# sisl/MADRL

Hardware: AMD Instinct MI355X
Metric: env-steps/sec at fixed batch (PursuitEvade 16x16, 8v30) (higher is better)
Workload: dtype u8/int32 grid state, f32 observations, f64 reward arithmetic; 1 GPU; PursuitEvade 16x16, 8 pursuers / 30 evaders, obs_range 7, rectangle_map, surround, n_catch 2, flatten, local reward, 65536 envs per GPU, horizon 500; envs_per_gpu=65536, envs_total=65536, parallelism=env-sharded x1, streams_per_gpu=2, rccl_ranks=1

## Files before the change

### madrl_amd/csrc/pursuit_wave.hpp

```cpp
#pragma once

#include <type_traits>

#include "common.hpp"

namespace madrl {
namespace pw {

#ifndef MADRL_PW_WAVES
#define MADRL_PW_WAVES 5
#endif
#define MADRL_PW_OCC __attribute__((amdgpu_waves_per_eu(S::OCC, S::OCC)))

constexpr uint32_t SENT = 0xFFFFFFFFu;
constexpr uint32_t CAUGHT = 0x10000u;

struct WaveDev {
    int32_t n_catch, surround, reward_global, sample_maps, n_maps, max_steps, auto_reset;
    int32_t fmap_stride;
    int32_t max_opponents;
    int32_t reverse;
    uint32_t k0, k1, gid_base;
    double catchr, term_pursuit, urgency, cw;
    int64_t n_envs;
    const uint32_t *fmaps;
    const float *vtab;
    const int32_t *pending;
    const uint32_t *cnt_tmpl;
    const uint32_t *slot_tab;
    const double *cw_env;
    const double *catchr_env;
    uint8_t *state;
    uint32_t *flags;
    uint32_t *zmask;
};

struct WaveIO {
    const uint8_t *mask;
    const int32_t *inj_pos;
    const int32_t *inj_map;
    const int32_t *actions;
    const int32_t *inj_eact;
    float *obs;
    float *rew;
    uint8_t *done;
    int32_t *removed;
    int32_t flex;
    int32_t control_evaders;
    const float *obs_prev;
};

__device__ __forceinline__ double sload_f64(const double *p, int64_t index) {
    return ((const __attribute__((address_space(4))) double *)(uint64_t)p)[index];
}

struct KArgs {
    WaveDev d;
    WaveIO io;
};
typedef const __attribute__((address_space(4))) KArgs *KArgsPtr;
__device__ __forceinline__ KArgsPtr cold_args() { return kernargs<KArgs>(); }
__device__ __forceinline__ int32_t pending_count(int64_t env, int k) {
    const int32_t *pend = cold_args()->d.pending;
    return ((const __attribute__((address_space(4))) int32_t *)(uint64_t)pend)[2 * env + k];
}

template <int XS_, int YS_, int P_, int E_, int R_, int FLATTEN_>
struct Shape {
    static constexpr int XS = XS_, YS = YS_, P = P_, E = E_, A = P_ + E_, R = R_, FLATTEN = FLATTEN_;
    static constexpr int OFF = (R - 1) / 2;
    static constexpr int PAD = OFF > 1 ? OFF : 1;
    static constexpr int GW = YS + 2 * PAD;
    static constexpr int GH = XS + 2 * PAD;
    static constexpr int GSZ = (GH * GW + 3) / 4 * 4;
    static constexpr int D = FLATTEN ? 3 * R * R + 1 : 4 * R * R;
    static constexpr int DV = D / 4;
    static constexpr int NQ = P * DV;
    static constexpr int NS = (NQ + 63) / 64;
    static constexpr int MWORDS = 1;
    static constexpr int OCC = NS <= 5 ? MADRL_PW_WAVES : (MADRL_PW_WAVES < 4 ? MADRL_PW_WAVES : 4);
    static constexpr int X_FILL = 3 * GSZ;
    static constexpr int X_SKIP = 3 * GSZ + 1;
    static constexpr int X_ID = 3 * GSZ + 2;
    static constexpr int X_VTAB = (X_ID + P + 3) / 4 * 4;
    static constexpr int NVT = 72;
    static constexpr int X_NEED = X_VTAB + NVT;
    static constexpr int X_OBSV = X_NEED + (XS * YS + 3) / 4;
    static constexpr int LDS_DWORDS = X_OBSV + (P + 3) / 4 * 4;
    static constexpr int NGW = (E + 31) / 32 > 0 ? (E + 31) / 32 : 1;
    static constexpr int NTW = (A + 31) / 32;
    static constexpr int OFF_GONE = (16 + 2 * A + 3) / 4 * 4;
    static constexpr int OFF_TERM = OFF_GONE + 4 * NGW;
    static constexpr int REC_BYTES = (OFF_TERM + 4 * NTW + 15) / 16 * 16;
    static constexpr int REC_DW = REC_BYTES / 4;
    static_assert(REC_DW <= 64, "the whole record must fit one dword per lane");
    static_assert(A <= 64, "one wavefront per env: n_pursuers + n_evaders must fit 64 lanes");
    static_assert(R % 2 == 1, "odd obs_range only (even ranges run on the generic kernel)");
    static_assert(D % 4 == 0, "observation row must be a whole number of float4");
    static_assert(LDS_DWORDS * 4 <= 64 * 1024, "LDS budget");
    static_assert(NS <= 8, "stale-zero mask: one bit per slot in each byte of the lane's mask dword");
    static constexpr bool LIVE = false;
    static constexpr bool TO = false;
    static constexpr bool TABLED = false;
    static constexpr int X_TAB = 0;
};

template <int XS_, int YS_, int P_, int E_, int R_, int FLATTEN_>
struct LShape : Shape<XS_, YS_, P_, E_, R_, FLATTEN_> {
    static constexpr bool LIVE = true;
};
constexpr int NOT_HERE = 0xFF;

template <int XS_, int YS_, int P_, int E_, int R_, int FLATTEN_>
struct TShape : Shape<XS_, YS_, P_, E_, R_, FLATTEN_> {
    static constexpr bool TO = true;
};
template <int XS_, int YS_, int P_, int E_, int R_, int FLATTEN_>
struct TLShape : LShape<XS_, YS_, P_, E_, R_, FLATTEN_> {
    static constexpr bool TO = true;
};

__device__ __forceinline__ double pairwise8(const double *r) {
    return ((r[0] + r[1]) + (r[2] + r[3])) + ((r[4] + r[5]) + (r[6] + r[7]));
}

template <int P>
__device__ __forceinline__ double np_sum_regs(const double (&a)[P]) {
    if constexpr (P < 8) {
        double res = 0.0;
#pragma unroll
        for (int i = 0; i < P; ++i) res += a[i];
        return res;
    } else {
        double r[8];
#pragma unroll
        for (int i = 0; i < 8; ++i) r[i] = a[i];
        constexpr int LIM = P - (P % 8);
#pragma unroll
        for (int i = 8; i < LIM; i += 8) {
#pragma unroll
            for (int k = 0; k < 8; ++k) r[k] += a[i + k];
        }
        double res = pairwise8(r);
#pragma unroll
        for (int i = LIM; i < P; ++i) res += a[i];
        return res;
    }
}

template <int P>
__device__ __forceinline__ double np_sum_first(const double (&a)[P], int n) {
    double res = 0.0;
    if (n < 8) {
#pragma unroll
        for (int i = 0; i < (P < 8 ? P : 7); ++i)
            if (i < n) res += a[i];
        return res;
    }
    if constexpr (P >= 8) {
        double r[8];
#pragma unroll
        for (int i = 0; i < 8; ++i) r[i] = a[i];
        const int lim = n - (n % 8);
#pragma unroll
        for (int i = 8; i + 8 <= P; i += 8) {
            if (i < lim) {
#pragma unroll
                for (int k = 0; k < 8; ++k) r[k] += a[i + k];
            }
        }
        res = pairwise8(r);
#pragma unroll
        for (int i = 8; i < P; ++i)
            if (i >= lim && i < n) res += a[i];
    }
    return res;
}

typedef float v4f_t __attribute__((ext_vector_type(4)));
template <int I, int N, class F>
__device__ __forceinline__ void static_for(F &&f) {
    if constexpr (I < N) {
        f(std::integral_constant<int, I>{});
        static_for<I + 1, N>(f);
    }
}
template <int OFF>
__device__ __forceinline__ void store_slot_masked(const void *base, uint32_t voff, uint32_t v0, uint32_t v1, uint32_t v2, uint32_t v3,
                                                  v4f_t val, uint64_t m0, uint64_t m1, uint64_t m2, uint64_t m3, uint64_t m_nt) {
    uint64_t sv;
    asm volatile("s_mov_b64 %0, exec\n\t"
                 "s_mov_b64 exec, %1\n\tglobal_store_dword %6, %7, %12 offset:%13\n\t"
                 "s_mov_b64 exec, %2\n\tglobal_store_dword %6, %8, %12 offset:%13+4\n\t"
                 "s_mov_b64 exec, %3\n\tglobal_store_dword %6, %9, %12 offset:%13+8\n\t"
                 "s_mov_b64 exec, %4\n\tglobal_store_dword %6, %10, %12 offset:%13+12\n\t"
                 "s_mov_b64 exec, %5\n\tglobal_store_dwordx4 %6, %11, %12 offset:%13 nt\n\t"
                 "s_mov_b64 exec, %0\n\ts_nop 0"
                 : "=&s"(sv) : "s"(m0), "s"(m1), "s"(m2), "s"(m3), "s"(m_nt), "v"(voff), "v"(v0), "v"(v1), "v"(v2), "v"(v3), "v"(val),
                   "s"(base), "n"(OFF));
}
__device__ __forceinline__ uint32_t quad_or(uint32_t v) {
    v |= (uint32_t)__builtin_amdgcn_update_dpp(0, (int)v, 0xB1, 0xF, 0xF, true);
    v |= (uint32_t)__builtin_amdgcn_update_dpp(0, (int)v, 0x4E, 0xF, 0xF, true);
    return v;
}

__device__ __forceinline__ void prefetch3(uint32_t &r0, uint32_t &r1, uint32_t &r2, const void *b0, uint32_t o0, const void *b1, uint32_t o1,
                                          const void *b2, uint32_t o2) {
    asm volatile("s_nop 4\n\tglobal_load_dword %0, %3, %4\n\tglobal_load_dword %1, %5, %6\n\tglobal_load_dword %2, %7, %8"
                 : "=&v"(r0), "=&v"(r1), "=&v"(r2) : "v"(o0), "s"(b0), "v"(o1), "s"(b1), "v"(o2), "s"(b2));
}
template <int N>
__device__ __forceinline__ void prefetch_wait(uint32_t &r0, uint32_t &r1, uint32_t &r2) {
    static_assert(N >= 0 && N < 64, "vmcnt is a 6-bit field");
    asm volatile("s_waitcnt vmcnt(%3)" : "+v"(r0), "+v"(r1), "+v"(r2) : "n"(N) : "memory");
}

template <int LN>
__device__ __forceinline__ void put_lane(uint32_t &w, uint32_t v) {
    const uint32_t sv = (uint32_t)__builtin_amdgcn_readfirstlane((int)v);
    asm("v_writelane_b32 %0, %1, %2" : "+v"(w) : "s"(sv), "n"(LN));
}
template <int LN, int END>
__device__ __forceinline__ void put_zero_from(uint32_t &w) {
    if constexpr (LN < END) {
        put_lane<LN>(w, 0u);
        put_zero_from<LN + 1, END>(w);
    }
}

template <class S, int NT>
struct Fill {
    static constexpr int NEEDW = (S::XS * S::YS + 3) / 4;
    static constexpr int TABW = S::TABLED ? 2 * S::DV : 0;
    static constexpr int J_MAP = (S::GSZ + NT - 1) / NT;
    static constexpr int J_NEED = 2 * J_MAP;
    static constexpr int J_VT = J_NEED + (NEEDW + NT - 1) / NT;
    static constexpr int J_TAB = J_VT + (S::NVT + NT - 1) / NT;
    static constexpr int J_END = J_TAB + (TABW + NT - 1) / NT;
    static constexpr int first(int j) { return j < J_MAP ? 0 : j < J_NEED ? J_MAP : j < J_VT ? J_NEED : j < J_TAB ? J_VT : J_TAB; }
    static constexpr int words(int j) { return j < J_NEED ? S::GSZ : j < J_VT ? NEEDW : j < J_TAB ? S::NVT : TABW; }
};
template <class S, int NT, int J>
__device__ __forceinline__ uint32_t fill_load(uint32_t utid, const uint32_t *cnt, const uint32_t *map, const uint32_t *vtab, const uint32_t *tab) {
    using F = Fill<S, NT>;
    constexpr int t = J - F::first(J), n = F::words(J);
    const uint32_t k = utid + (uint32_t)(NT * t);
    const uint32_t kc = (NT * (t + 1) <= n) ? k : (k < (uint32_t)n ? k : (uint32_t)n - 1u);
    if constexpr (J < F::J_MAP) return cnt[kc];
    else if constexpr (J < F::J_NEED) return map[kc];
    else if constexpr (J < F::J_VT) return map[(uint32_t)S::GSZ + kc];
    else if constexpr (J < F::J_TAB) return vtab[kc];
    else return tab[kc];
}
template <class S, int NT, int J, bool FIRST>
__device__ __forceinline__ void fill_store(uint32_t *L, uint32_t utid, uint32_t v) {
    using F = Fill<S, NT>;
    constexpr int t = J - F::first(J), n = F::words(J);
    const uint32_t k = utid + (uint32_t)(NT * t);
    if ((NT * (t + 1) <= n) || k < (uint32_t)n) {
        if constexpr (J < F::J_MAP) {
            L[S::GSZ + k] = v;
            L[2 * S::GSZ + k] = v;
        } else if constexpr (J < F::J_NEED) L[k] = v;
        else if constexpr (J < F::J_VT) L[S::X_NEED + k] = v;
        else if constexpr (J < F::J_TAB) L[S::X_VTAB + k] = v;
        else L[S::X_TAB + k] = v;
    }
    if constexpr (FIRST && J == F::J_MAP) {
        if (utid == 0u) {
            L[S::X_FILL] = v;
            L[S::X_SKIP] = SENT;
        }
    }
}
template <int N>
__device__ __forceinline__ void staged_wait(uint32_t *a) {
    if constexpr (N >= 8) {
        asm volatile("" : "+v"(a[N - 1]), "+v"(a[N - 2]), "+v"(a[N - 3]), "+v"(a[N - 4]), "+v"(a[N - 5]), "+v"(a[N - 6]), "+v"(a[N - 7]), "+v"(a[N - 8]));
        staged_wait<N - 8>(a);
    } else if constexpr (N >= 4) {
        asm volatile("" : "+v"(a[N - 1]), "+v"(a[N - 2]), "+v"(a[N - 3]), "+v"(a[N - 4]));
        staged_wait<N - 4>(a);
    } else if constexpr (N >= 2) {
        asm volatile("" : "+v"(a[N - 1]), "+v"(a[N - 2]));
        staged_wait<N - 2>(a);
    } else if constexpr (N == 1) {
        asm volatile("" : "+v"(a[0]));
    }
}
template <class S, int NT, int J0, int J1, int CAP, bool FIRST>
__device__ __forceinline__ void fill_trips(uint32_t *L, uint32_t utid, const uint32_t *cnt, const uint32_t *map, const uint32_t *vtab, const uint32_t *tab) {
    if constexpr (J0 < J1) {
        constexpr int JB = J0 + CAP < J1 ? J0 + CAP : J1;
        uint32_t st[JB - J0];
        static_for<J0, JB>([&](auto jc) {
            if constexpr (decltype(jc)::value == JB - 1) __builtin_amdgcn_sched_barrier(0);
            st[decltype(jc)::value - J0] = fill_load<S, NT, decltype(jc)::value>(utid, cnt, map, vtab, tab);
        });
        staged_wait<JB - J0>(st);
        static_for<J0, JB>([&](auto jc) { fill_store<S, NT, decltype(jc)::value, FIRST>(L, utid, st[decltype(jc)::value - J0]); });
        fill_trips<S, NT, JB, J1, CAP, FIRST>(L, utid, cnt, map, vtab, tab);
    }
}
constexpr int FILL_FIRST = 56, FILL_BATCH = 16;

#ifndef MADRL_ABLATE
#define MADRL_ABLATE 0
#endif
#ifndef MADRL_PW_EXP
#define MADRL_PW_EXP 0
#endif

template <class S, int MODE, bool INJECT, bool CTRL = false>
__global__ __launch_bounds__(64) MADRL_PW_OCC void pursuit_wave_kernel(const WaveDev d, const WaveIO io) {
    static_assert(!CTRL || (S::E >= S::P && (MODE == 0 || INJECT)), "evader control: n_evaders >= n_pursuers, flexible instantiation");
    static_assert(!CTRL || !S::LIVE, "evader control has no per-env agent counts");
    static_assert(!S::TO || (MODE == 1 && INJECT && !CTRL), "the two-buffer step: the flexible step kernel only");
    constexpr int P = S::P, E = S::E, A = S::A, GW = S::GW, PAD = S::PAD, GSZ = S::GSZ, NS = S::NS;
    __shared__ __attribute__((aligned(16))) uint32_t L[S::LDS_DWORDS];
    const int lane = threadIdx.x;
    const uint32_t ulane = threadIdx.x;
    const bool is_p = lane < P;
    const int eslot = lane - P;

#if MADRL_PW_EXP & 4
    if (d.n_envs > 0) return;
#endif
    using F = Fill<S, 64>;
    const int n_envs = (int)d.n_envs, stride = (int)gridDim.x;
    if (n_envs <= 0) return;
    auto phys = [&](int e) -> int64_t { return (int64_t)(d.reverse ? n_envs - 1 - e : e); };
    const uint32_t *const vtab_u = reinterpret_cast<const uint32_t *>(d.vtab);
    constexpr int ROOM = FILL_FIRST - 6 * NS - 3;
    constexpr int JF = F::J_END < (ROOM > 4 ? ROOM : 4) ? F::J_END : (ROOM > 4 ? ROOM : 4);
    const uint32_t rec_off = (ulane < (uint32_t)S::REC_DW ? ulane : (uint32_t)S::REC_DW - 1u) * 4u;
    const uint32_t act_off = (ulane < (uint32_t)P ? ulane : (uint32_t)P - 1u) * 4u;
    uint32_t st[JF], sraw[6 * NS];
    static_for<0, JF>([&](auto jc) { st[decltype(jc)::value] = fill_load<S, 64, decltype(jc)::value>(ulane, d.cnt_tmpl, d.fmaps, vtab_u, nullptr); });
#pragma unroll
    for (int k = 0; k < 6 * NS; ++k) sraw[k] = d.slot_tab[64u * k + ulane];
    uint32_t cur_rec, cur_zm;
    int cur_act = 4;
    __builtin_amdgcn_sched_barrier(0);
    {
        const int64_t env0 = phys((int)blockIdx.x < n_envs ? (int)blockIdx.x : n_envs - 1);
        cur_rec = *reinterpret_cast<const uint32_t *>(d.state + env0 * (int64_t)S::REC_BYTES + rec_off);
        if constexpr (MODE == 1) cur_act = *reinterpret_cast<const int *>(reinterpret_cast<const char *>(io.actions + env0 * P) + act_off);
        cur_zm = d.zmask[env0 * 64 + ulane];
    }
    asm volatile("" : "+v"(cur_rec), "+v"(cur_act), "+v"(cur_zm));
    staged_wait<6 * NS>(sraw);
    staged_wait<JF>(st);
    static_for<0, JF>([&](auto jc) { fill_store<S, 64, decltype(jc)::value, true>(L, ulane, st[decltype(jc)::value]); });
    fill_trips<S, 64, JF, F::J_END, FILL_BATCH, true>(L, ulane, d.cnt_tmpl, d.fmaps, vtab_u, nullptr);
    if (lane < P) L[S::X_ID + lane] = __float_as_uint((float)((double)lane / (double)P));
    if (ulane >= (uint32_t)S::REC_DW) cur_rec = 0u;
    if (!is_p) cur_act = 4;
    int s_cst[NS][4];
    int s_rel3[NS];
    int s_src[NS];
#pragma unroll
    for (int s = 0; s < NS; ++s) {
#pragma unroll
        for (int k = 0; k < 4; ++k) s_cst[s][k] = (int)sraw[6 * s + k] * 4;
        s_rel3[s] = (int)sraw[6 * s + 4];
        s_src[s] = (int)sraw[6 * s + 5] * 4;
    }
    int cached_map = 0;
    int cached_np = P;
    const uint8_t *need_tab = reinterpret_cast<const uint8_t *>(&L[S::X_NEED]);
    uint32_t *const layer = &L[is_p ? GSZ : 2 * GSZ];
    const int rec_src0 = (lane >= 4 ? 2 * (lane - 4) : 0) * 4, rec_src1 = rec_src0 + 4;

    auto isP = [&]() { return fresh(lane) < P; };
    auto isE = [&]() { return (unsigned)(fresh(lane) - P) < (unsigned)E; };
    auto isAgent = [&]() { return fresh(lane) < A; };
    auto fetch_rec = [&](int64_t env) -> uint32_t {
        return (fresh(lane) < S::REC_DW) ? uniform_ptr(reinterpret_cast<const uint32_t *>(d.state + env * (int64_t)S::REC_BYTES))[ulane] : 0u;
    };
    auto fetch_act = [&](int64_t env) -> int {
        if constexpr (MODE == 1) return isP() ? uniform_ptr(io.actions + env * P)[ulane] : 4;
        else return 4;
    };
    auto fetch_zm = [&](int64_t env) -> uint32_t { return uniform_ptr(d.zmask + env * 64)[ulane]; };
    wave_sync();
#if MADRL_PW_EXP & 8
    if (d.n_envs > 0) { if (s_cst[0][0] + s_cst[NS - 1][3] + s_rel3[0] + s_src[NS - 1] + (int)cur_rec == 0x12345) io.rew[0] = 1.f; return; }
#endif

    constexpr bool PIPE = (MODE == 1) && !INJECT && !(MADRL_ABLATE & (1 | 8 | 16 | 64));
    constexpr int VM_PER_ENV = 5 * NS + 6;
    static_assert(!PIPE || VM_PER_ENV < 64, "vmcnt range");
    for (int e = blockIdx.x; e < n_envs; e += stride) {
        const int64_t env = phys(e);
        const bool has_next = e + stride < n_envs;
        const int64_t nenv = phys(has_next ? e + stride : e);
        uint32_t nxt_rec = 0, nxt_zm = 0xFFFFFFFFu;
        int nxt_act = 4;
        uint32_t pf_rec, pf_act, pf_zm;
        if constexpr (PIPE) {
            prefetch3(pf_rec, pf_act, pf_zm, d.state + nenv * (int64_t)S::REC_BYTES, rec_off, io.actions + nenv * P, act_off,
                      d.zmask + nenv * 64, ulane * 4u);
        } else {
#if MADRL_ABLATE & 64
            nxt_rec = cur_rec ^ (uint32_t)(fresh(lane) == 0);
            nxt_act = cur_act;
#else
            if (has_next) {
                nxt_rec = fetch_rec(nenv);
                nxt_act = fetch_act(nenv);
                nxt_zm = fetch_zm(nenv);
            }
#endif
        }
        bool skip = false;
        if constexpr (MODE == 0) skip = (io.mask != nullptr && io.mask[env] == 0);
        if (!skip) {
            uint32_t tick = __builtin_amdgcn_readlane(cur_rec, 0);
            int32_t tstep = (int32_t)__builtin_amdgcn_readlane(cur_rec, 1);
            int32_t map_id = (int32_t)__builtin_amdgcn_readlane(cur_rec, 2);
            const uint32_t xyw = (uint32_t)__shfl((int)cur_rec, 4 + (lane >> 1));
            const uint32_t xy = (lane & 1) ? (xyw >> 16) : (xyw & 0xFFFFu);
            int x = (int)(xy & 0xFF), y = (int)(xy >> 8);
            uint64_t gone = (uint32_t)__builtin_amdgcn_readlane(cur_rec, S::OFF_GONE / 4);
            if constexpr (S::NGW > 1) gone |= (uint64_t)(uint32_t)__builtin_amdgcn_readlane(cur_rec, S::OFF_GONE / 4 + 1) << 32;
            uint64_t term = (uint32_t)__builtin_amdgcn_readlane(cur_rec, S::OFF_TERM / 4);
            if constexpr (S::NTW > 1) term |= (uint64_t)(uint32_t)__builtin_amdgcn_readlane(cur_rec, S::OFF_TERM / 4 + 1) << 32;
            const uint32_t gid = d.gid_base + (uint32_t)env;
            const uint32_t k0 = fresh_s(d.k0), k1 = fresh_s(d.k1);
            int np = P, ne = E;
            if constexpr (S::LIVE) {
                const bool here = x != NOT_HERE;
                np = __popcll(__builtin_amdgcn_ballot_w64(isP() && here));
                ne = __popcll(__builtin_amdgcn_ballot_w64(isE() && here));
                if (!here) {
                    x = 0;
                    y = 0;
                }
            }
            auto isLP = [&]() {
                if constexpr (S::LIVE) return fresh(lane) < np;
                else return isP();
            };
            bool do_reset = (MODE == 0);
            uint32_t done_bits = 0;
            float rew_out = 0.0f;
            int n_removed = 0;
            bool alive = isLP() || (isE() && !((gone >> eslot) & 1ull));
            int cell = (x + PAD) * GW + y + PAD;

            auto load_map = [&](int mid) {
                if (cached_map == mid) return;
                const KArgsPtr ka = cold_args();
                fill_trips<S, 64, F::J_MAP, F::J_VT, FILL_BATCH, false>(L, ulane, nullptr, ka->d.fmaps + (int64_t)mid * ka->d.fmap_stride, nullptr, nullptr);
                cached_map = mid;
                wave_sync();
            };
            load_map(map_id);

            if constexpr (MODE == 1) {
                const bool e_alive = alive && !isP();
                if (e_alive) atomicAdd(&layer[cell], 1u);
                wave_sync();
                int kpre = 0;
                if (isP()) {
                    const int dxm = (x > 0) ? GW : 0, dxp = (x < S::XS - 1) ? GW : 0;
                    const int dym = (y > 0) ? 1 : 0, dyp = (y < S::YS - 1) ? 1 : 0;
                    const uint32_t *ec = &L[2 * GSZ];
                    kpre = (int)(ec[cell - dxm] + ec[cell + dxp] + ec[cell + dyp] + ec[cell - dym]);
                }
                wave_sync();
                if (e_alive) atomicSub(&layer[cell], 1u);
                const int kidx = __popcll((~gone) & ((1ull << (eslot & 63)) - 1ull));
                int act = cur_act;
                bool injected = false;
                if constexpr (CTRL) {
                    const int from_k = __builtin_amdgcn_ds_bpermute((kidx < P ? kidx : 0) * 4, cur_act);
                    injected = io.inj_eact != nullptr;
                    int pact;
                    if (injected) pact = isP() ? io.inj_eact[env * P + lane] : 4;
                    else pact = (int)__umulhi(philox4x32_10(gid, tick, (uint32_t)lane, TAG_PURSUER_ACT, k0, k1).x, 5u);
                    act = isP() ? pact : (kidx < P ? from_k : 4);
                    injected = true;
                } else if constexpr (INJECT) {
                    injected = io.inj_eact != nullptr;
                    if (injected && e_alive) act = io.inj_eact[env * E + kidx];
                }
                if (!injected) {
#if MADRL_ABLATE & 4
                    u32x4 r; r.x = (gid * 2654435761u + tick * 40503u + (uint32_t)kidx * 2246822519u) ^ k0 ^ k1;
#else
                    const u32x4 r = philox4x32_10(gid, tick, (uint32_t)kidx, TAG_EVADER_ACT, k0, k1);
#endif
                    if (!isP()) act = (int)__umulhi(r.x, 5u);
                }
                const int dcell = (act == 0 ? -GW : 0) + (act == 1 ? GW : 0) + (act == 2 ? 1 : 0) + (act == 3 ? -1 : 0);
                const bool tflag = (term >> lane) & 1ull;
                const bool in_building = L[cell] != 0u;
                const bool target_free = L[cell + dcell] == 0u;
                const bool newterm = alive && !tflag && in_building;
                if (alive && !tflag && !in_building && target_free) {
                    cell += dcell;
                    x += (act == 1) - (act == 0);
                    y += (act == 2) - (act == 3);
                }
                term |= __ballot(newterm);
                if (alive) atomicAdd(&layer[cell], 1u);
                wave_sync();
                bool caught = false;
                if (e_alive) {
                    const uint32_t *pc = &L[GSZ];
                    if (d.surround) {
                        const uint32_t n0 = pc[cell - GW], n1 = pc[cell + GW], n2 = pc[cell + 1], n3 = pc[cell - 1];
                        const int cnt = (int)(n0 - 1u < SENT - 1u) + (int)(n1 - 1u < SENT - 1u) +
                                        (int)(n2 - 1u < SENT - 1u) + (int)(n3 - 1u < SENT - 1u);
                        caught = cnt == (int)need_tab[x * S::YS + y];
                    } else {
                        caught = (int)pc[cell] >= d.n_catch;
                    }
                    if (caught) atomicAdd(&layer[cell], CAUGHT);
                }
                const uint64_t caught_mask = __ballot(caught) >> P;
                gone |= caught_mask;
                wave_sync();
                double r = 0.0;
                if (isLP()) {
                    const uint32_t *ec = &L[2 * GSZ];
                    bool sur;
                    if (d.surround) {
                        const uint32_t n0 = ec[cell - GW], n1 = ec[cell + GW], n2 = ec[cell + 1], n3 = ec[cell - 1];
                        sur = ((n0 != SENT) & (n0 >= CAUGHT)) | ((n1 != SENT) & (n1 >= CAUGHT)) |
                              ((n2 != SENT) & (n2 >= CAUGHT)) | ((n3 != SENT) & (n3 >= CAUGHT));
                    } else {
                        sur = ec[cell] >= CAUGHT;
                    }
                    double catchr = d.catchr;
                    if constexpr (INJECT) { if (d.catchr_env != nullptr) catchr = sload_f64(d.catchr_env, env); }
                    r = catchr * (double)kpre;
                    r += d.term_pursuit * (sur ? 1.0 : 0.0);
                    r += d.urgency;
                }
                if (d.reward_global) {
                    double all[P];
#pragma unroll
                    for (int k = 0; k < P; ++k) all[k] = __shfl(r, k);
                    if constexpr (S::LIVE) r = isLP() ? np_sum_first<P>(all, np) / (double)np : 0.0;
                    else r = np_sum_regs<P>(all) / (double)P;
                }
                tick += 1;
                tstep += 1;
                constexpr uint64_t all_e = (1ull << E) - 1ull;
                if ((gone & all_e) == all_e) done_bits |= 1u;
                if (d.max_steps > 0 && tstep >= d.max_steps) done_bits |= 2u;
                do_reset = d.auto_reset && done_bits != 0;
                rew_out = (float)r;
                n_removed = __popcll(caught_mask);
            }

            if constexpr (!PIPE) asm volatile("" : "+v"(nxt_rec), "+v"(nxt_act), "+v"(nxt_zm));
            uint32_t zm = cur_zm;

            const int npass = (MODE == 1 && do_reset) ? 2 : 1;
            for (int pass = 0; pass < npass; ++pass) {
                if (do_reset && pass == npass - 1) {
                    gone = 0ull;
                    term = 0ull;
                    const KArgsPtr ka = cold_args();
                    const double cw = ka->d.cw_env != nullptr ? sload_f64(ka->d.cw_env, env) : ka->d.cw;
                    const int max_opponents = ka->d.max_opponents;
                    bool inj_map = false, inj_pos = false;
                    if constexpr (MODE == 0) {
                        inj_map = io.inj_map != nullptr;
                        inj_pos = io.inj_pos != nullptr;
                    }
                    if (inj_map) {
                        map_id = __builtin_amdgcn_readfirstlane(io.inj_map[env]);
                    } else if (ka->d.sample_maps) {
                        const u32x4 rm = philox4x32_10(gid, tick, 0u, TAG_RESET_ENV, k0, k1);
                        map_id = (int)__umulhi(rm.x, (uint32_t)ka->d.n_maps);
                    }
                    load_map(map_id);
                    const u32x4 rw = philox4x32_10(gid, tick, 1u, TAG_RESET_ENV, k0, k1);
                    const double sx = u53(rw.x, rw.y) * (1.0 - cw);
                    const double sy = u53(rw.z, rw.w) * (1.0 - cw);
                    const int xlb = (int)(S::XS * sx), xub = (int)(S::XS * (sx + cw));
                    const int ylb = (int)(S::YS * sy), yub = (int)(S::YS * (sy + cw));
                    int n_create = E;
                    if constexpr (S::LIVE) {
                        np = min(max(pending_count(env, 0), 1), P);
                        ne = min(max(pending_count(env, 1), 0), E);
                        n_create = ne;
                    }
                    if (max_opponents > 0 && !inj_pos) {
                        const u32x4 r3 = philox4x32_10(gid, tick, 2u, TAG_RESET_ENV, k0, k1);
                        n_create = min(1 + (int)__umulhi(r3.x, (uint32_t)(max_opponents - 1)), S::LIVE ? ne : E);
                    }
                    bool exists = false;
                    if (isAgent()) {
                        if constexpr (S::LIVE) exists = isLP() || (!isP() && eslot < n_create);
                        else exists = isP() || eslot < n_create;
                        if (inj_pos) {
                            x = io.inj_pos[(env * A + lane) * 2];
                            y = io.inj_pos[(env * A + lane) * 2 + 1];
                            if (!isP() && x < 0) exists = false;
                        } else {
                            for (uint32_t att = 0; att < 1024u; ++att) {
                                const uint32_t aidx = S::LIVE ? (uint32_t)(isP() ? lane : np + eslot) : (uint32_t)lane;
                                const u32x4 rp = philox4x32_10(gid, tick, aidx, TAG_RESET_POS | (att << 8), k0, k1);
                                x = xlb + (int)__umulhi(rp.x, (uint32_t)(xub - xlb));
                                y = ylb + (int)__umulhi(rp.y, (uint32_t)(yub - ylb));
                                if (L[(x + PAD) * GW + y + PAD] == 0u) break;
                            }
                        }
                        if (exists) {
                            cell = (x + PAD) * GW + y + PAD;
                            atomicAdd(&layer[cell], 1u);
                        } else {
                            x = 0;
                            y = 0;
                        }
                    }
                    gone = __ballot(isE() && !exists) >> P;
                    alive = exists;
                    tick += 1;
                    tstep = 0;
                    wave_sync();
                }
                if constexpr (S::LIVE) {
                    if (np != cached_np) {
                        if (lane < P) L[S::X_ID + lane] = __float_as_uint((float)((double)lane / (double)np));
                        cached_np = np;
                        wave_sync();
                    }
                }
                uint32_t cnt = 0;
                if (alive) cnt = layer[cell] & 0xFFFFu;
                wave_sync();
                if (alive) layer[cell] = L[S::X_VTAB + cnt];
                wave_sync();
#if MADRL_ABLATE & 8
                if (d.n_envs < 0)
#endif
                {
                    int origin = isP() ? ((x - S::OFF + PAD) * GW + (y - S::OFF + PAD)) * 4 : 0;
                    int n_rows = P;
                    if constexpr (CTRL) {
                        const uint64_t obsv = ~gone & ((1ull << P) - 1ull);
                        n_rows = __popcll(obsv);
                        const bool is_obs = isE() && eslot < P && ((obsv >> (eslot & 63)) & 1ull);
                        if (is_obs) L[S::X_OBSV + __popcll(obsv & ((1ull << (eslot & 63)) - 1ull))] = (uint32_t)(((x - S::OFF + PAD) * GW + (y - S::OFF + PAD)) * 4);
                        wave_sync();
                        origin = (isP() && lane < n_rows) ? (int)L[S::X_OBSV + lane] : 0;
                    }
                    if constexpr (S::LIVE) n_rows = np;
                    const char *orow_u = (const char *)uniform_ptr(io.obs + env * (int64_t)(P * S::D));
                    asm volatile("s_nop 4" : "+s"(orow_u));
                    const uint32_t voff = ulane * 16u;
                    [[maybe_unused]] const auto prow_g = uniform_ptr(S::TO ? io.obs_prev + env * (int64_t)(P * S::D) : io.obs);
                    [[maybe_unused]] const auto orow_g = uniform_ptr(io.obs + env * (int64_t)(P * S::D));
                    const char *Lb = reinterpret_cast<const char *>(L);
                    auto cell_at = [&](int off) -> uint32_t { return *reinterpret_cast<const uint32_t *>(Lb + off); };
                    uint32_t acc = 0u;
                    [[maybe_unused]] uint32_t to_need[S::TO ? NS : 1], to_bits[S::TO ? NS : 1];
                    static_for<0, NS>([&](auto sc) {
                        constexpr int s = decltype(sc)::value;
                        const int base = __builtin_amdgcn_ds_bpermute(s_src[s], origin);
                        const uint32_t v0 = cell_at(base + s_cst[s][0]);
                        const uint32_t v1 = cell_at(base + s_cst[s][1]);
                        const uint32_t v2 = cell_at(base + s_cst[s][2]);
                        const uint32_t v3 = cell_at((int)__umul24((uint32_t)base, (uint32_t)s_rel3[s]) + s_cst[s][3]);
                        const uint32_t top = __builtin_amdgcn_perm(v1, v0, 0x0C0C0703u) | __builtin_amdgcn_perm(v3, v2, 0x07030C0Cu);
                        const uint32_t out4 = (top >> 7) & 0x01010101u;
                        const uint32_t nz4 = ((top >> 5) | (top >> 6)) & 0x01010101u;
                        const uint32_t old4 = (zm >> (NS - 1 - s)) & 0x01010101u;
                        const uint32_t dirty = out4 & old4;
                        if constexpr (S::TO) {
                            if (pass == 0) {
                                bool row_live = true;
                                if constexpr (S::LIVE) row_live = (s_src[s] >> 2) < n_rows;
                                const bool in_row = (64 * (s + 1) <= S::NQ) ? true : (fresh(lane) + 64 * s < S::NQ);
                                const uint32_t need4 = in_row ? (row_live ? dirty : 0x01010101u) : 0u;
                                to_need[s] = need4;
                                to_bits[s] = ~need4 & ~out4 & nz4;
                                return;
                            }
                        }
                        bool valid = (64 * (s + 1) <= S::NQ) ? true : (fresh(lane) + 64 * s < S::NQ);
                        if constexpr (CTRL || S::LIVE) {
                            const bool row_live = (s_src[s] >> 2) < n_rows;
                            acc = (acc << 1) | (row_live ? ((out4 & old4) | (~out4 & nz4)) : old4);
                            valid = valid && row_live;
                        } else {
                            acc = (acc << 1) | ((out4 & old4) | (~out4 & nz4));
                        }
                        bool clean = dirty == 0u;
#if MADRL_ABLATE & 1
                        valid = d.n_envs < 0;
#endif
#if MADRL_ABLATE & 2
                        clean = true;
#endif
                        const uint32_t st = valid ? (clean ? 0u : dirty) : 0x80000000u;
#if MADRL_ABLATE & 32
                        {
                            uint32_t burn = acc;
                            asm volatile("v_xor_b32 %0, %0, %1\n v_xor_b32 %0, %0, %1\n v_xor_b32 %0, %0, %1\n v_xor_b32 %0, %0, %1\n v_xor_b32 %0, %0, %1\n"
                                         "v_xor_b32 %0, %0, %1\n v_xor_b32 %0, %0, %1\n v_xor_b32 %0, %0, %1\n v_xor_b32 %0, %0, %1\n v_xor_b32 %0, %0, %1\n"
                                         "v_xor_b32 %0, %0, %1\n v_xor_b32 %0, %0, %1\n v_xor_b32 %0, %0, %1\n v_xor_b32 %0, %0, %1\n v_xor_b32 %0, %0, %1\n"
                                         "v_xor_b32 %0, %0, %1\n v_xor_b32 %0, %0, %1\n v_xor_b32 %0, %0, %1\n v_xor_b32 %0, %0, %1\n v_xor_b32 %0, %0, %1"
                                         : "+v"(burn) : "v"(v0));
                            acc = burn;
                        }
#endif
#if MADRL_ABLATE & 128
                        {
                            uint32_t sburn = fresh_s(0u);
                            asm volatile("s_add_u32 %0, %0, 1\n s_add_u32 %0, %0, 1\n s_add_u32 %0, %0, 1\n s_add_u32 %0, %0, 1\n s_add_u32 %0, %0, 1\n"
                                         "s_add_u32 %0, %0, 1\n s_add_u32 %0, %0, 1\n s_add_u32 %0, %0, 1\n s_add_u32 %0, %0, 1\n s_add_u32 %0, %0, 1\n"
                                         "s_add_u32 %0, %0, 1\n s_add_u32 %0, %0, 1\n s_add_u32 %0, %0, 1\n s_add_u32 %0, %0, 1\n s_add_u32 %0, %0, 1\n"
                                         "s_add_u32 %0, %0, 1\n s_add_u32 %0, %0, 1\n s_add_u32 %0, %0, 1\n s_add_u32 %0, %0, 1\n s_add_u32 %0, %0, 1"
                                         : "+s"(sburn) : : "scc");
                        }
#endif
                        const void *sb = orow_u + 4096 * (s / 4);
                        const uint32_t lim = (uint32_t)fresh((st - 1u < 0x01010101u) ? (int)SENT : 0);
                        const uint32_t grp = quad_or(st == 0u ? (out4 ^ 0x01010101u) : 0u);
                        const uint32_t nt = (uint32_t)fresh(st == 0u ? (int)grp : 0);
                        const v4f_t val = {__uint_as_float((uint32_t)max((int)v0, 0)), __uint_as_float((uint32_t)max((int)v1, 0)),
                                           __uint_as_float((uint32_t)max((int)v2, 0)), __uint_as_float((uint32_t)max((int)v3, 0))};
                        store_slot_masked<1024 * (s % 4)>(sb, voff, v0, v1, v2, v3, val, __builtin_amdgcn_ballot_w64(v0 < lim),
                                                          __builtin_amdgcn_ballot_w64(v1 < lim), __builtin_amdgcn_ballot_w64(v2 < lim),
                                                          __builtin_amdgcn_ballot_w64(v3 < lim), __builtin_amdgcn_ballot_w64(nt != 0u));
                    });
                    if constexpr (S::TO) {
                        if (pass == 0) {
                            typedef uint32_t v4u_t __attribute__((ext_vector_type(4)));
                            typedef __attribute__((address_space(1))) v4u_t gv4u_t;
                            typedef __attribute__((address_space(1))) v4f_t gv4f_t;
                            constexpr int TG = NS <= 5 ? NS : 4;
                            auto emit = [&](auto sc, const v4u_t oldv) {
                                constexpr int s = decltype(sc)::value;
                                const int base = __builtin_amdgcn_ds_bpermute(s_src[s], origin);
                                const uint32_t need4 = to_need[s];
                                uint32_t w0 = (uint32_t)max((int)cell_at(base + s_cst[s][0]), 0);
                                uint32_t w1 = (uint32_t)max((int)cell_at(base + s_cst[s][1]), 0);
                                uint32_t w2 = (uint32_t)max((int)cell_at(base + s_cst[s][2]), 0);
                                uint32_t w3 = (uint32_t)max((int)cell_at((int)__umul24((uint32_t)base, (uint32_t)s_rel3[s]) + s_cst[s][3]), 0);
                                if (need4 & 0x00000001u) w0 = oldv.x;
                                if (need4 & 0x00000100u) w1 = oldv.y;
                                if (need4 & 0x00010000u) w2 = oldv.z;
                                if (need4 & 0x01000000u) w3 = oldv.w;
                                const uint32_t oldnz = (oldv.x != 0u ? 0x00000001u : 0u) | (oldv.y != 0u ? 0x00000100u : 0u) |
                                                       (oldv.z != 0u ? 0x00010000u : 0u) | (oldv.w != 0u ? 0x01000000u : 0u);
                                acc = (acc << 1) | to_bits[s] | (need4 & oldnz);
                                const bool in_row = (64 * (s + 1) <= S::NQ) ? true : (fresh(lane) + 64 * s < S::NQ);
                                if (in_row) {
                                    const v4f_t wv = {__uint_as_float(w0), __uint_as_float(w1), __uint_as_float(w2), __uint_as_float(w3)};
                                    __builtin_nontemporal_store(wv, reinterpret_cast<gv4f_t *>(orow_g) + (64u * s + ulane));
                                }
                            };
                            static_for<0, (NS + TG - 1) / TG>([&](auto gc) {
                                constexpr int g0 = decltype(gc)::value * TG, g1 = g0 + TG < NS ? g0 + TG : NS;
                                uint32_t any = 0u;
#pragma unroll
                                for (int s = g0; s < g1; ++s) any |= to_need[s];
                                if (__builtin_amdgcn_ballot_w64(any != 0u) != 0ull) {
                                    v4u_t old[TG];
#pragma unroll
                                    for (int s = g0; s < g1; ++s) {
                                        old[s - g0] = v4u_t{0u, 0u, 0u, 0u};
                                        if (to_need[s] != 0u) old[s - g0] = reinterpret_cast<const gv4u_t *>(prow_g)[64u * s + ulane];
                                    }
                                    static_for<g0, g1>([&](auto sc) { emit(sc, old[decltype(sc)::value - g0]); });
                                } else {
                                    static_for<g0, g1>([&](auto sc) { emit(sc, v4u_t{0u, 0u, 0u, 0u}); });
                                }
                            });
                        }
                    }
                    zm = acc;
                }
                wave_sync();
                if (alive) layer[cell] = 0u;
                wave_sync();
            }
#if MADRL_ABLATE & 16
            if (d.n_envs < 0)
#endif
            if constexpr (MODE == 1) {
                if (isP()) uniform_ptr(io.rew + env * P)[ulane] = rew_out;
                if (fresh(lane) == 0) {
                    io.done[env] = (uint8_t)done_bits;
                    io.removed[env] = n_removed;
                    cold_args()->d.flags[env] = done_flag_word(done_bits);
                }
            }
            {
                int myxy = x | (y << 8);
                if constexpr (S::LIVE) {
                    if (!(isP() ? isLP() : eslot < ne)) myxy = NOT_HERE | (NOT_HERE << 8);
                }
                const uint32_t lo = (uint32_t)__builtin_amdgcn_ds_bpermute(rec_src0, myxy);
                const uint32_t hi = (uint32_t)__builtin_amdgcn_ds_bpermute(rec_src1, myxy);
                uint32_t w = (lo & 0xFFFFu) | (hi << 16);
                put_lane<0>(w, tick);
                put_lane<1>(w, (uint32_t)tstep);
                put_lane<2>(w, (uint32_t)map_id);
                put_lane<3>(w, 0u);
                put_lane<S::OFF_GONE / 4>(w, (uint32_t)gone);
                if constexpr (S::NGW > 1) put_lane<S::OFF_GONE / 4 + 1>(w, (uint32_t)(gone >> 32));
                put_lane<S::OFF_TERM / 4>(w, (uint32_t)term);
                if constexpr (S::NTW > 1) put_lane<S::OFF_TERM / 4 + 1>(w, (uint32_t)(term >> 32));
                put_zero_from<S::OFF_TERM / 4 + S::NTW, S::REC_DW>(w);
#if MADRL_ABLATE & 16
                if (d.n_envs < 0)
#endif
                if (fresh(lane) < S::REC_DW)
                    uniform_ptr(reinterpret_cast<uint32_t *>(d.state + env * (int64_t)S::REC_BYTES))[ulane] = w;
#if MADRL_ABLATE & 16
                if (d.n_envs < 0)
#endif
                uniform_ptr(d.zmask + env * 64)[ulane] = zm;
            }
        }
        if constexpr (PIPE) {
            prefetch_wait<VM_PER_ENV>(pf_rec, pf_act, pf_zm);
            nxt_rec = (fresh(lane) < S::REC_DW) ? pf_rec : 0u;
            nxt_act = (int)pf_act;
            nxt_zm = pf_zm;
        }
        cur_rec = nxt_rec;
        cur_act = nxt_act;
        cur_zm = nxt_zm;
    }
}

template <class S>
void wave_to_launch(const WaveDev &d, const WaveIO &io, int64_t blocks, hipStream_t s);

}
}
```

Baseline: 1.142 billion env-steps/s.

## Pack per-env zmask into 16 bits per lane to halve its traffic

Adds a compressed zmask layout for flatten observations: each lane's mask bits for useful observation slots are packed into 16 bits, and two lanes share one dword, so each env stores 32 dwords instead of 64. Loads fetch the shared dword and unpack it by half-wave. Stores pack the mask and combine lane halves with a permlane32 swap. The aim is to cut global read and write bytes per env step, at the cost of a few extra ALU/permute ops, and it relies on the eligibility analysis that never-useful slots can be dropped.

```diff
diff --git a/madrl_amd/csrc/pursuit_wave.hpp b/madrl_amd/csrc/pursuit_wave.hpp
--- a/madrl_amd/csrc/pursuit_wave.hpp
+++ b/madrl_amd/csrc/pursuit_wave.hpp
@@ -3,6 +3,7 @@
 #include <type_traits>
 
 #include "common.hpp"
+#include "pursuit_zm16.hpp"
 
 namespace madrl {
 namespace pw {
@@ -78,6 +79,8 @@
     static constexpr int NQ = P * DV;
     static constexpr int NS = (NQ + 63) / 64;
     static constexpr int MWORDS = 1;
+    static constexpr bool ZM16 = zm16::eligible(P, R, FLATTEN);
+    static constexpr int ZMW = ZM16 ? 32 : 64;
     static constexpr int OCC = NS <= 5 ? MADRL_PW_WAVES : (MADRL_PW_WAVES < 4 ? MADRL_PW_WAVES : 4);
     static constexpr int X_FILL = 3 * GSZ;
     static constexpr int X_SKIP = 3 * GSZ + 1;
@@ -331,6 +334,9 @@
     const int n_envs = (int)d.n_envs, stride = (int)gridDim.x;
     if (n_envs <= 0) return;
     auto phys = [&](int e) -> int64_t { return (int64_t)(d.reverse ? n_envs - 1 - e : e); };
+    auto zm_env = [](int64_t env) -> int64_t { return (MADRL_ABLATE & (256 | 512)) ? (env & 255) : env; };
+    const uint32_t zm_lane = S::ZM16 ? (ulane & 31u) : ulane;
+    [[maybe_unused]] const uint32_t zm_keep = S::ZM16 ? zm16::keep_low(P, S::R, lane) : 0u;
     const uint32_t *const vtab_u = reinterpret_cast<const uint32_t *>(d.vtab);
     constexpr int ROOM = FILL_FIRST - 6 * NS - 3;
     constexpr int JF = F::J_END < (ROOM > 4 ? ROOM : 4) ? F::J_END : (ROOM > 4 ? ROOM : 4);
@@ -347,7 +353,7 @@
         const int64_t env0 = phys((int)blockIdx.x < n_envs ? (int)blockIdx.x : n_envs - 1);
         cur_rec = *reinterpret_cast<const uint32_t *>(d.state + env0 * (int64_t)S::REC_BYTES + rec_off);
         if constexpr (MODE == 1) cur_act = *reinterpret_cast<const int *>(reinterpret_cast<const char *>(io.actions + env0 * P) + act_off);
-        cur_zm = d.zmask[env0 * 64 + ulane];
+        cur_zm = d.zmask[zm_env(env0) * S::ZMW + zm_lane];
     }
     asm volatile("" : "+v"(cur_rec), "+v"(cur_act), "+v"(cur_zm));
     staged_wait<6 * NS>(sraw);
@@ -383,14 +389,14 @@
         if constexpr (MODE == 1) return isP() ? uniform_ptr(io.actions + env * P)[ulane] : 4;
         else return 4;
     };
-    auto fetch_zm = [&](int64_t env) -> uint32_t { return uniform_ptr(d.zmask + env * 64)[ulane]; };
+    auto fetch_zm = [&](int64_t env) -> uint32_t { return uniform_ptr(d.zmask + zm_env(env) * S::ZMW)[zm_lane]; };
     wave_sync();
 #if MADRL_PW_EXP & 8
     if (d.n_envs > 0) { if (s_cst[0][0] + s_cst[NS - 1][3] + s_rel3[0] + s_src[NS - 1] + (int)cur_rec == 0x12345) io.rew[0] = 1.f; return; }
 #endif
 
     constexpr bool PIPE = (MODE == 1) && !INJECT && !(MADRL_ABLATE & (1 | 8 | 16 | 64));
-    constexpr int VM_PER_ENV = 5 * NS + 6;
+    constexpr int VM_PER_ENV = 5 * NS + 6 - ((MADRL_ABLATE & 512) ? 1 : 0);
     static_assert(!PIPE || VM_PER_ENV < 64, "vmcnt range");
     for (int e = blockIdx.x; e < n_envs; e += stride) {
         const int64_t env = phys(e);
@@ -401,7 +407,7 @@
         uint32_t pf_rec, pf_act, pf_zm;
         if constexpr (PIPE) {
             prefetch3(pf_rec, pf_act, pf_zm, d.state + nenv * (int64_t)S::REC_BYTES, rec_off, io.actions + nenv * P, act_off,
-                      d.zmask + nenv * 64, ulane * 4u);
+                      d.zmask + zm_env(nenv) * S::ZMW, zm_lane * 4u);
         } else {
 #if MADRL_ABLATE & 64
             nxt_rec = cur_rec ^ (uint32_t)(fresh(lane) == 0);
@@ -560,6 +566,7 @@
 
             if constexpr (!PIPE) asm volatile("" : "+v"(nxt_rec), "+v"(nxt_act), "+v"(nxt_zm));
             uint32_t zm = cur_zm;
+            if constexpr (S::ZM16) zm = zm16::unpack(fresh(lane) < 32 ? cur_zm : cur_zm >> 16, zm_keep);
 
             const int npass = (MODE == 1 && do_reset) ? 2 : 1;
             for (int pass = 0; pass < npass; ++pass) {
@@ -698,7 +705,7 @@
 #if MADRL_ABLATE & 1
                         valid = d.n_envs < 0;
 #endif
-#if MADRL_ABLATE & 2
+#if MADRL_ABLATE & (2 | 512)
                         clean = true;
 #endif
                         const uint32_t st = valid ? (clean ? 0u : dirty) : 0x80000000u;
@@ -821,7 +828,15 @@
 #if MADRL_ABLATE & 16
                 if (d.n_envs < 0)
 #endif
-                uniform_ptr(d.zmask + env * 64)[ulane] = zm;
+#if !(MADRL_ABLATE & 512)
+                if constexpr (S::ZM16) {
+                    const uint32_t h = zm16::pack(zm, zm_keep);
+                    const uint32_t other = __builtin_amdgcn_permlane32_swap(h, h, false, false)[1];
+                    if (fresh(lane) < 32) uniform_ptr(d.zmask + zm_env(env) * S::ZMW)[ulane] = h | (other << 16);
+                } else {
+                    uniform_ptr(d.zmask + zm_env(env) * 64)[ulane] = zm;
+                }
+#endif
             }
         }
         if constexpr (PIPE) {
diff --git a/madrl_amd/csrc/pursuit_zm16.hpp b/madrl_amd/csrc/pursuit_zm16.hpp
--- /dev/null
+++ b/madrl_amd/csrc/pursuit_zm16.hpp
@@ -0,0 +1,81 @@
+#pragma once
+
+#include <stdint.h>
+
+#if defined(__HIPCC__)
+#define MADRL_ZM16_HD __host__ __device__
+#else
+#define MADRL_ZM16_HD
+#endif
+
+namespace madrl {
+namespace zm16 {
+
+constexpr int LANES = 64;
+
+constexpr int row_slots(int R, int flatten) { return (flatten ? 3 * R * R + 1 : 4 * R * R) / 4; }
+constexpr int lane_slots(int P, int R, int flatten) { return (P * row_slots(R, flatten) + LANES - 1) / LANES; }
+
+MADRL_ZM16_HD constexpr bool useful(int P, int R, int q) {
+    const int dv = row_slots(R, 1), m = q % dv;
+    return q < P * dv && 4 * m + 3 >= R * R && 4 * m < 3 * R * R;
+}
+MADRL_ZM16_HD constexpr int useful_slots(int P, int R, int lane) {
+    int n = 0;
+    for (int s = 0; s < lane_slots(P, R, 1); ++s) n += useful(P, R, lane + LANES * s) ? 1 : 0;
+    return n;
+}
+constexpr bool eligible(int P, int R, int flatten) {
+    if (flatten != 1 || lane_slots(P, R, 1) > 5) return false;
+    for (int lane = 0; lane < LANES; ++lane)
+        if (useful_slots(P, R, lane) > 4) return false;
+    return true;
+}
+MADRL_ZM16_HD constexpr int drop_slot(int P, int R, int lane) {
+    const int ns = lane_slots(P, R, 1);
+    int d = -1;
+    for (int s = 0; s < (ns == 5 ? ns : 0); ++s)
+        if (!useful(P, R, lane + LANES * s)) d = s;
+    return d;
+}
+MADRL_ZM16_HD constexpr uint32_t keep_low(int P, int R, int lane) {
+    const int ns = lane_slots(P, R, 1);
+    if (ns != 5) return 0x0F0F0F0Fu;
+    return 0x01010101u * ((1u << (ns - 1 - drop_slot(P, R, lane))) - 1u);
+}
+MADRL_ZM16_HD constexpr uint32_t useful_bits(int P, int R, int lane) {
+    const int ns = lane_slots(P, R, 1);
+    uint32_t u = 0u;
+    for (int s = 0; s < ns; ++s)
+        if (useful(P, R, lane + LANES * s)) u |= 0x01010101u << (ns - 1 - s);
+    return u;
+}
+
+MADRL_ZM16_HD inline uint32_t perm(uint32_t hi, uint32_t lo, uint32_t sel) {
+#if defined(__HIP_DEVICE_COMPILE__)
+    return __builtin_amdgcn_perm(hi, lo, sel);
+#else
+    uint32_t r = 0u;
+    for (int k = 0; k < 4; ++k) {
+        const uint32_t c = (sel >> (8 * k)) & 0xFFu;
+        const uint32_t b = c < 4u ? (lo >> (8 * c)) & 0xFFu : c < 8u ? (hi >> (8 * (c - 4u))) & 0xFFu : 0u;
+        r |= b << (8 * k);
+    }
+    return r;
+#endif
+}
+MADRL_ZM16_HD inline uint32_t bfi(uint32_t m, uint32_t a, uint32_t b) { return (a & m) | (b & ~m); }
+
+MADRL_ZM16_HD inline uint32_t pack(uint32_t x, uint32_t keep) {
+    const uint32_t n = bfi(keep, x, x >> 1) & 0x0F0F0F0Fu;
+    const uint32_t t = n | (n >> 4);
+    return perm(0u, t, 0x0C0C0200u);
+}
+MADRL_ZM16_HD inline uint32_t unpack(uint32_t h, uint32_t keep) {
+    const uint32_t t = perm(0u, h, 0x0C010C00u);
+    const uint32_t n = (t | (t << 4)) & 0x0F0F0F0Fu;
+    return bfi(keep, n, n << 1);
+}
+
+}
+}
```

Result: faster. 1.191 billion env-steps/s (median of 6 runs) (+4.3%).
